# libertininick/imagescry

Hardware: AMD Instinct MI355X
Metric: queries/s cosine top-10 over N x D bank (higher is better)
Workload: dtype f16; 1 GPU; cosine top-10: 1024 fp16 queries x 10000000 x 768 fp16 bank (BASELINE config 4 bank; row-sharded 1 way); bank_rows=10000000, dim=768, queries=1024, k=10, rows_per_gpu=10000000, parallelism=row-shard1

## Files before the change

### imagescry_amd/_lib.py

```python

from __future__ import annotations

import ctypes
import math
import os
from ctypes import POINTER, c_char_p, c_float, c_int, c_int32, c_int64, c_size_t, c_void_p
from pathlib import Path

import torch

LIB_NAME = "libimagescry_hip.so"
LIB_PATH = Path(os.environ.get("ISC_LIB") or Path(__file__).resolve().parent / LIB_NAME)

ISC_U8, ISC_F16, ISC_F32 = 0, 1, 2
ISC_ACT_NONE, ISC_ACT_RELU, ISC_ACT_GELU, ISC_ACT_SILU, ISC_ACT_SIGMOID = 0, 1, 2, 3, 4
ISC_ACT_RESIDUAL_AFTER = 0x100
ISC_TOPK_MAX_K = 120
ISC_SEARCH_MAX_D = 8192
ISC_SEARCH_PASS_QUERIES = 1024
ISC_ABI_VERSION = 4
ISC_BUILD_ABLATION = 1
ISC_GEMM_A_PACKED, ISC_GEMM_W_PACKED, ISC_GEMM_OUT_PACKED, ISC_GEMM_TILE_256, ISC_GEMM_TILE_128 = 1, 2, 4, 8, 16
ISC_KERNEL_DOTS_FILTER, ISC_KERNEL_CONV, ISC_KERNEL_GEMM_F16 = 0, 1, 2

# ... 111 lines not shown
    "isc_im2col_nchw": (
        c_int,
        [c_void_p, c_int, c_int, c_int, c_int, c_int, c_int, c_int, c_int, c_int, c_void_p, c_void_p],
    ),
    "isc_maxpool_nhwc": (c_int, [c_void_p, c_int, c_int, c_int, c_int, c_int, c_int, c_int, c_void_p, c_void_p]),
    "isc_global_avgpool_nhwc": (c_int, [c_void_p, c_int, c_int, c_int, c_int, c_void_p, c_void_p]),
    "isc_pool_linear_l2norm": (
        c_int, [c_void_p, c_int, c_int, c_int, c_int, c_void_p, c_void_p, c_int, c_int, c_float, c_void_p, c_void_p]
    ),
    "isc_gemm_f16": (
        c_int,
        [c_void_p, c_int64, c_int, c_void_p, c_int, c_void_p, c_void_p, c_int, c_void_p, c_int, c_int, c_void_p],
    ),
    "isc_layernorm": (
        c_int,
        [c_void_p, c_int64, c_int, c_int64, c_void_p, c_void_p, c_float, c_void_p, c_int, c_int64, c_int, c_void_p],
    ),
    "isc_attention_f16": (c_int, [c_void_p, c_int, c_int, c_int, c_int, c_void_p, c_int, c_void_p]),
    "isc_patchify_f16": (c_int, [c_void_p, c_int, c_int, c_int, c_int, c_int, c_void_p, c_int, c_void_p]),
    "isc_vit_assemble": (c_int, [c_void_p, c_void_p, c_void_p, c_int, c_int, c_int, c_void_p, c_void_p]),
    "isc_vit_pos_resample": (c_int, [c_void_p, c_int, c_int, c_int, c_int, c_void_p, c_void_p]),
    "isc_vit_tokens_out": (
        c_int, [c_void_p, c_int, c_int, c_int, c_void_p, c_void_p, c_float, c_int, c_float, c_void_p, c_void_p]
    ),
    "isc_cosine_topk_workspace_bytes": (c_int, [c_int, c_int64, c_int, c_int, c_int, POINTER(c_size_t)]),
    "isc_cosine_topk": (
        c_int,
        [c_void_p, c_int, c_int64, c_int, c_void_p, c_int, c_int, c_int64, c_int, c_int64, c_void_p, c_void_p, c_void_p,
         c_void_p, c_void_p, c_size_t, c_void_p],
    ),
    "isc_bank_shadow_bytes": (c_int, [c_int64, c_int, POINTER(c_size_t)]),
    "isc_bank_quantize": (c_int, [c_void_p, c_int64, c_int, c_void_p, c_size_t, c_void_p]),
    "isc_cosine_topk_uses_shadow": (c_int, [c_int, c_int64, c_int, c_int, c_int, POINTER(c_int)]),
    "isc_cosine_topk_shadow": (
        c_int,
        [c_void_p, c_int, c_int64, c_int, c_void_p, c_int, c_int, c_int64, c_int, c_int64, c_void_p, c_void_p, c_void_p,
         c_void_p, c_void_p, c_size_t, c_void_p, c_void_p],
    ),
    "isc_cosine_topk_exhaustive_workspace_bytes": (c_int, [c_int, c_int64, c_int, c_int, c_int, POINTER(c_size_t)]),
    "isc_cosine_topk_exhaustive": (
        c_int,
        [c_void_p, c_int, c_int64, c_int, c_void_p, c_int, c_int, c_int64, c_int, c_int64, c_void_p, c_void_p,
         c_void_p, c_size_t, c_void_p],
    ),
    "isc_cosine_range_workspace_bytes": (c_int, [c_int, c_int64, c_int, c_int, c_int64, POINTER(c_size_t)]),
    "isc_cosine_range": (
        c_int,
        [c_void_p, c_int, c_int64, c_int, c_void_p, c_int, c_int, c_int64, c_void_p, c_int64, c_void_p, c_int64,
         c_void_p, c_void_p, c_void_p, c_void_p, c_void_p, c_void_p, c_size_t, c_void_p],
    ),
    "isc_row_mask_words": (c_int, [c_int64, POINTER(c_size_t)]),
    "isc_row_mask_pack": (c_int, [c_void_p, c_int64, c_void_p, c_void_p, c_void_p]),
    "isc_row_mask_unpack": (c_int, [c_void_p, c_int64, c_int64, c_void_p, c_void_p]),
    "isc_cosine_topk_masked": (
        c_int,
        [c_void_p, c_int, c_int64, c_int, c_void_p, c_int, c_int, c_int64, c_int, c_int64, c_void_p, c_void_p, c_void_p,
         c_void_p, c_void_p, c_size_t, c_void_p, c_void_p],
    ),
    "isc_cosine_topk_exhaustive_masked": (
        c_int,
        [c_void_p, c_int, c_int64, c_int, c_void_p, c_int, c_int, c_int64, c_int, c_int64, c_void_p, c_void_p,
         c_void_p, c_size_t, c_void_p, c_void_p],
    ),
    "isc_cosine_range_masked": (
        c_int,
        [c_void_p, c_int, c_int64, c_int, c_void_p, c_int, c_int, c_int64, c_void_p, c_int64, c_void_p, c_int64,
# ... 130 lines not shown
```

### imagescry_amd/csrc/cosine_topk.hip

```cpp
#include <math.h>
#include <stdlib.h>

#include <type_traits>

#include "bank_layout.h"
#include "isc_common.h"
#include "search_common.h"

namespace {

typedef _Float16 half8 __attribute__((ext_vector_type(8)));
typedef float f32x4 __attribute__((ext_vector_type(4)));
typedef unsigned u32x4 __attribute__((ext_vector_type(4)));
typedef int i32x4 __attribute__((ext_vector_type(4)));

constexpr int TM = 256;
constexpr int NTHREADS = 512;
constexpr int CAP = 32;
constexpr int TARGET_WGS = 256;
constexpr int QCAP = 8192;
constexpr int SLACK = 6;
constexpr int SMALL_Q = 128;
constexpr int QBATCH = ISC_SEARCH_PASS_QUERIES;
constexpr int MAX_LEVELS = 12;
constexpr int SEL_THREADS = 512;
constexpr int SURV_CAP = 2048;
constexpr int TAIL_LCAP = 256;
constexpr int TAIL_COUNT_OFF = 64 * TAIL_LCAP * 8;
constexpr int TAIL_LBOUND_OFF = 140 * 1024;

struct Cand {
    float s;
    int32_t row;
};

struct Level {
    int64_t r0, r1;
    int ntiles, tiles_per_chunk, nchunks;
    int sample;
};

struct Plan {
    int tnq;
    int segs_per_chunk;
    int kp;
    int nslots;
    int qb;
    int qtiles;
    int qpad;
    int max_seg;
    int nlevels;
    int64_t budget;
    Level levels[MAX_LEVELS];
};

int plan_kp(int k) { return (int)isc_align_up((size_t)k + SLACK, 16); }

#ifdef ISC_ABLATION
int forced_tile() {
    static const int v = [] {
        const char* e = getenv("ISC_FORCE_TILE");
        return e ? atoi(e) : 0;
    }();
    return v;
}
#else
constexpr int forced_tile() { return 0; }
#endif

#ifdef ISC_ABLATION
__device__ int g_abl_thr_inf = 0;
int first_ratio() {
    static const int v = getenv("ISC_FIRST_RATIO") ? atoi(getenv("ISC_FIRST_RATIO")) : 16;
    return v;
}
int sample_tiles_cap() {
    static const int v = getenv("ISC_SAMPLE_TILES") ? atoi(getenv("ISC_SAMPLE_TILES")) : 0;
    return v;
}
#else
constexpr int first_ratio() { return 16; }
constexpr int sample_tiles_cap() { return 0; }
#endif

constexpr int COLLAPSE_MIN_KP = 32;
constexpr int COLLAPSE_ROWS_CAP = 64;
constexpr int COLLAPSE_GROUPS = 4096;

Plan make_plan(int64_t n, int q, int k, int group_rows = 0) {
    Plan p;
    p.qb = q < QBATCH ? q : QBATCH;
    p.tnq = p.qb <= 64 ? 64 : p.qb <= SMALL_Q ? 128 : 256;
    if (forced_tile() == 64 || forced_tile() == 128 || forced_tile() == 256) p.tnq = forced_tile();
    p.segs_per_chunk = (8 / (p.tnq / 64)) * 4;
    p.kp = plan_kp(k);
    if (group_rows > 0 && p.kp < COLLAPSE_MIN_KP) p.kp = COLLAPSE_MIN_KP;
    p.qtiles = isc_ceil_div(p.qb, p.tnq);
    p.qpad = p.qtiles * p.tnq;
    p.nslots = group_rows > 0 ? 0 : p.kp <= 16 ? 32 : p.kp <= 32 ? 64 : p.kp <= 64 ? 128 : 0;
    int wgs = TARGET_WGS / p.qtiles;
    if (wgs < 1) wgs = 1;
    const int64_t ntiles_all = isc_ceil_div<int64_t>(n, TM);

    p.nlevels = 0;
    p.max_seg = 0;
    p.budget = 0;
    auto add = [&](int64_t r0, int64_t r1, int sample) {
        Level& l = p.levels[p.nlevels++];
        l.r0 = r0;
        l.r1 = r1;
        l.sample = sample;
        l.ntiles = (int)isc_ceil_div<int64_t>(r1 - r0, TM);
        int want = sample ? l.ntiles : wgs;
        if (want > l.ntiles) want = l.ntiles;
        l.tiles_per_chunk = isc_ceil_div(l.ntiles, want);
        l.nchunks = isc_ceil_div(l.ntiles, l.tiles_per_chunk);
        if (p.segs_per_chunk * l.nchunks > p.max_seg) p.max_seg = p.segs_per_chunk * l.nchunks;
    };
    int64_t stiles = p.nslots ? (int64_t)(QCAP * 7 / 10) / (p.kp * 27 / 20) : 16;
    if (stiles > wgs) stiles = wgs;
    if (sample_tiles_cap() > 0 && stiles > sample_tiles_cap()) stiles = sample_tiles_cap();
    if (stiles < 1) stiles = 1;
    if (stiles > ntiles_all) stiles = ntiles_all;
    int64_t seen = stiles * TM < n ? stiles * TM : n;
    add(0, seen, 1);
    while (seen < n) {
        const int64_t nseg = (int64_t)p.segs_per_chunk * wgs;
        int64_t budget = (int64_t)((double)QCAP * p.kp / (p.kp + 8.0 * sqrt((double)p.kp)));
        if (group_rows > 0) budget = (int64_t)((double)COLLAPSE_GROUPS * p.kp / (p.kp + 8.0 * sqrt((double)p.kp)));
        if (nseg * CAP / 8 < budget) budget = nseg * CAP / 8;
        p.budget = budget;
        const int64_t unit = (int64_t)p.kp * (group_rows > COLLAPSE_ROWS_CAP ? COLLAPSE_ROWS_CAP : group_rows > 0 ? group_rows : 1);
        int64_t ratio = 1 + budget / unit;
        if (p.tnq == 256 && p.qtiles == 1 && p.nlevels == 1 && ratio > first_ratio()) ratio = first_ratio();
        if (ratio < 3) ratio = 3;
        int64_t r1 = seen * ratio;
        if (r1 > n || p.nlevels == MAX_LEVELS - 1) r1 = n;
        add(seen, r1, 0);
        seen = r1;
    }
    const int redo_chunks = (int)(wgs < ntiles_all ? wgs : ntiles_all);
    if (p.segs_per_chunk * redo_chunks > p.max_seg) p.max_seg = p.segs_per_chunk * redo_chunks;
    return p;
}

struct Workspace {
    float* tau;
    float* carry_s;
    int32_t* carry_r;
    int32_t* carry_n;
    int32_t* qflag;
    Cand* seg_ent;
    int32_t* qcount;
    Cand* qlist;
    unsigned char* qpacked;
    int32_t* r_count;
    int32_t* r_list;
    float* tau2;
    int32_t* qcount2;
    int32_t* qflag2;
    unsigned char* qpacked2;
    IscExactWs exact;
    unsigned char* qpacked8;
    float4* qrec8;
    size_t bytes;
};

Workspace carve(const Plan& p, int ks, int64_t n, int k, void* base) {
    Workspace w;
    size_t off = 0;
    auto take = [&](size_t bytes) {
        void* ptr = base ? static_cast<char*>(base) + off : nullptr;
// ... 152 lines not shown
    }
    static __device__ __forceinline__ void row(const u32x4& a0, const u32x4& a1, const u32x4 (&b)[2][4],
                                               f32x4 (&acc)[4]) {
        half(a0, b[0], acc);
        half(a1, b[1], acc);
    }
    template <int N0, int N1>
    static __device__ __forceinline__ void part(const u32x4& a, const u32x4 (&b)[4], f32x4 (&acc)[4]) {
#pragma unroll
        for (int j = 0; j < 4; ++j)
#pragma unroll
            for (int n = N0; n < N1; ++n)
                acc[n] = __builtin_amdgcn_mfma_f32_16x16x4f32(__uint_as_float(a[j]), __uint_as_float(b[n][j]), acc[n],
                                                              0, 0, 0);
    }
};

template <>
struct Mma<signed char> {
    typedef i32x4 Acc;
    template <int N0, int N1>
    static __device__ __forceinline__ void part(const u32x4& a, const u32x4 (&b)[4], i32x4 (&acc)[4]) {
#pragma unroll
        for (int n = N0; n < N1; ++n)
            acc[n] = __builtin_amdgcn_mfma_i32_16x16x64_i8(__builtin_bit_cast(i32x4, a), __builtin_bit_cast(i32x4, b[n]),
                                                           acc[n], 0, 0, 0);
    }
};

struct IscShadowArgs {
    const IscShadowRec* recs;
    const float4* qrec;
};

#define ISC_DS_READ(dst_, addr_, off_) \
    asm volatile("ds_read_b128 %0, %1 offset:%2" : "=v"(dst_) : "v"(addr_), "i"(off_))

__device__ __forceinline__ void glds16(const unsigned char* gsrc, unsigned char* lds_wave_base) {
    __builtin_amdgcn_global_load_lds((const __attribute__((address_space(1))) void*)gsrc,
                                     (__attribute__((address_space(3))) void*)lds_wave_base, 16, 0, 0);
}
template <bool NT>
__device__ __forceinline__ void glds16_bank(const unsigned char* gsrc, unsigned char* lds_wave_base) {
    if constexpr (NT)
        __builtin_amdgcn_global_load_lds((const __attribute__((address_space(1))) void*)gsrc,
                                         (__attribute__((address_space(3))) void*)lds_wave_base, 16, 0, 2);
    else
        glds16(gsrc, lds_wave_base);
}

template <int N>
__device__ __forceinline__ void wait_vmcnt() {
    static_assert(N >= 0 && N <= 63, "vmcnt range");
    asm volatile("s_waitcnt vmcnt(%0)" ::"i"(N) : "memory");
}

constexpr int A_TILE_BYTES = TM * 128;

#ifndef ISC_ASYM_MBLO
#define ISC_ASYM_MBLO 6
#endif
#ifndef ISC_ASYM_SPLIT_MBLO
#define ISC_ASYM_SPLIT_MBLO 8
#endif
#ifndef ISC_HM_RING
#define ISC_HM_RING 4
// ... 566 lines not shown
            asm volatile("s_waitcnt lgkmcnt(0)" : "+v"(ar[cur_][0]), "+v"(ar[cur_][1]));                            \
        __builtin_amdgcn_sched_barrier(0);                                                                           \
        if constexpr (MODE != 3)                                                                                      \
            Mma<T>::row(ar[cur_][0], ar[cur_][1], bq, acc[m_]);                                                      \
        else                                                                                                         \
            acc[m_][0][0] += __uint_as_float(ar[cur_][0][0] ^ ar[cur_][1][1] ^ bq[0][1][0] ^ bq[1][2][1]);           \
    }
            ISC_ROW_STEP(0, 0, 1)
            ISC_ROW_STEP(1, 1, 0)
            ISC_ROW_STEP(2, 0, 1)
            ISC_ROW_STEP(3, 1, 0)
            ISC_ROW_STEP(4, 0, 1)
            ISC_ROW_STEP(5, 1, 0)
            ISC_ROW_STEP(6, 0, 1)
            ISC_ROW_STEP(7, 1, 0)
#undef ISC_ROW_STEP
            }
        }

        }

        if constexpr (!SAMPLE) {
        if (++kt == ksteps) {
            kt = 0;
            constexpr int MBE = STAGGER ? MBHI : MBLO;
            const int64_t trow0 = r0 + (int64_t)(tile_begin + tile) * TM + wave_row0 + fg * 4;
            if constexpr (MASK) {
                if (use_mask) apply_mask(MBE_C{}, SUB_C{}, tile_mask);
            }
            if constexpr (GROUP && !DEFER) apply_codes(MBE_C{}, tile_codes);
            if constexpr (I8) {
                int thr_i[4];
#pragma unroll
                for (int n = 0; n < 4; ++n) {
                    const float t = thr[n] * tile_ct;
                    const float mg = fmaf(qn8[n], tile_et, eq8[n] * (tile_nt + tile_et));
                    const float lo = (t - mg) - (fabsf(t) + mg) * 9.5367431640625e-7f - 1e-30f;
                    thr_i[n] = !(lo <= 2.0e9f) ? INT32_MAX : lo < -2.0e9f ? INT32_MIN : (int)floorf(lo);
                    if (!(tile_nt < INFINITY)) thr_i[n] = thr[n] < INFINITY ? INT32_MIN : INT32_MAX;
                }
                if (r0 + (int64_t)(tile_begin + tile + 1) * TM > r1) {
#pragma unroll
                    for (int m = 0; m < MBE; ++m)
#pragma unroll
                        for (int r = 0; r < 4; ++r)
                            if (trow0 + m * 16 + r >= r1) {
#pragma unroll
                                for (int n = 0; n < 4; ++n) acc[m][n][r] = INT32_MIN;
                            }
                }
#pragma unroll
                for (int n = 0; n < 4; ++n) {
                    int bm[MBE];
                    int mx = INT32_MIN;
#pragma unroll
                    for (int m = 0; m < MBE; ++m) {
                        bm[m] = max(max(acc[m][n][0], acc[m][n][1]), max(acc[m][n][2], acc[m][n][3]));
                        mx = max(mx, bm[m]);
                    }
                    if (__ballot(mx > thr_i[n]) != 0ull) {
#pragma unroll
                        for (int m = 0; m < MBE; ++m) {
                            if (__ballot(bm[m] > thr_i[n]) == 0ull) continue;
#pragma unroll
                            for (int r = 0; r < 4; ++r) {
                                if (acc[m][n][r] > thr_i[n]) {
                                    const int pos = cnt[n]++;
                                    if (pos < CAP)
                                        my_ent[n * 16 * CAP + pos] = Cand{(float)acc[m][n][r], (int32_t)(trow0 + m * 16 + r)};
                                }
                            }
                        }
                    }
// ... 332 lines not shown
}

template <int SPEC>
__global__ __launch_bounds__(SEL_THREADS, 4) void k_select(int32_t* __restrict__ qcount, const Cand* __restrict__ qlist,
                                                        int kp, float* __restrict__ tau, float* __restrict__ carry_s,
                                                        int32_t* __restrict__ carry_r, int32_t* __restrict__ carry_n,
                                                        int32_t* __restrict__ qflag) {
    __shared__ SelShared sh;
    const int q = blockIdx.x;
    const int n = wg_select<SPEC>(sh, q, kp, qcount, qlist, carry_s, carry_r, carry_n);
    const int tid = threadIdx.x;
    if (n < 0) {
        if (tid == 0) {
            qflag[q] = 1;
            tau[q] = INFINITY;
            carry_n[q] = 0;
            qcount[q] = 0;
        }
        return;
    }
    if (tid < n) {
        const unsigned long long key = sh.topk[tid];
        const float sc = isc_key_score(key);
        carry_s[(size_t)q * kp + tid] = sc;
        carry_r[(size_t)q * kp + tid] = isc_key_row(key);
        if (tid == kp - 1) tau[q] = sc;
    }
    if (tid == 0) {
        carry_n[q] = n;
        qcount[q] = 0;
    }
}

__global__ __launch_bounds__(SEL_THREADS, 2) void k_rescore(const unsigned char* __restrict__ bank, int ks,
                                                            const unsigned char* __restrict__ qpacked, int tnq,
                                                            const float* __restrict__ tau, int32_t* __restrict__ qcount,
                                                            Cand* __restrict__ qlist, int64_t nrows) {
    __shared__ float score[QCAP];
    __shared__ int kept;
    const int q = blockIdx.x;
    const int tid = threadIdx.x, lane = tid & 63, wave = tid >> 6;
    constexpr int NW = SEL_THREADS / 64;
    const int n = min(qcount[q], QCAP);
    Cand* list = qlist + (size_t)q * QCAP;
    const unsigned char* qrow_base = qpacked + ((size_t)(q / tnq) * ks * tnq + (q % tnq)) * ISC_KSTEP_BYTES;
    const int nch = ks * 8;
    float qv[2][8];
#pragma unroll
    for (int h = 0; h < 2; ++h) {
        const int ch = lane + 64 * h;
        uint4 raw = make_uint4(0u, 0u, 0u, 0u);
        if (ch < nch) raw = *reinterpret_cast<const uint4*>(qrow_base + (size_t)(ch >> 3) * tnq * ISC_KSTEP_BYTES + (ch & 7) * 16);
        const _Float16* hv = reinterpret_cast<const _Float16*>(&raw);
#pragma unroll
        for (int j = 0; j < 8; ++j) qv[h][j] = (float)hv[j];
    }
    if (tid == 0) kept = 0;
    for (int c0 = wave; c0 < n; c0 += 4 * NW) {
        float acc[4];
#pragma unroll
        for (int u = 0; u < 4; ++u) {
            const int c = c0 + u * NW;
            int row = c < n ? list[c].row : 0;
            if ((unsigned)row >= (unsigned)nrows) row = 0;
            acc[u] = 0.f;
#pragma unroll
            for (int h = 0; h < 2; ++h) {
                const int ch = lane + 64 * h;
                if (ch < nch) {
                    const uint4 raw = *reinterpret_cast<const uint4*>(bank + isc_packed_offset(row, ch >> 3, ks) + (ch & 7) * 16);
                    const _Float16* hv = reinterpret_cast<const _Float16*>(&raw);
#pragma unroll
                    for (int j = 0; j < 8; ++j) acc[u] = fmaf((float)hv[j], qv[h][j], acc[u]);
                }
            }
        }
#pragma unroll
        for (int u = 0; u < 4; ++u) {
            const float tot = isc_wave_sum(acc[u]);
            if (lane == 0 && c0 + u * NW < n) score[c0 + u * NW] = tot;
        }
    }
    __syncthreads();
    const float t = tau[q];
    int rows[SEL_PER];
#pragma unroll
    for (int j = 0; j < SEL_PER; ++j) rows[j] = tid + SEL_THREADS * j < n ? list[tid + SEL_THREADS * j].row : 0;
    __syncthreads();
#pragma unroll
    for (int j = 0; j < SEL_PER; ++j) {
        const int i = tid + SEL_THREADS * j;
        if (i < n && score[i] > t) list[atomicAdd(&kept, 1)] = Cand{score[i], rows[j]};
    }
    __syncthreads();
    if (tid == 0) qcount[q] = kept;
}

template <typename T, typename RowOf, typename Store>
__device__ void exact_dots(const unsigned char* __restrict__ bank, int ks, const unsigned char* qrow_base, int tnq,
                           int nc, int64_t nrows, RowOf row_of, Store store) {
    const int lane = threadIdx.x & 63, wave = threadIdx.x >> 6;
    const int sub = lane >> 3, ch = lane & 7;
    constexpr int NW = SEL_THREADS / 64;
    for (int c0 = wave; c0 < nc; c0 += 4 * NW) {
        int row[4];
        double acc[4];
#pragma unroll
        for (int u = 0; u < 4; ++u) {
            const int c = c0 + u * NW;
            row[u] = c < nc ? row_of(c) : -1;
            if ((unsigned)row[u] >= (unsigned)nrows) row[u] = -1;
            acc[u] = 0.0;
        }
        for (int s0 = 0; s0 < ks; s0 += 8) {
            const int s = s0 + sub;
            if (s < ks) {
                double a[4][8], b[8];
#pragma unroll
                for (int u = 0; u < 4; ++u)
                    Chunk16<T>::load(bank + isc_packed_offset(row[u] < 0 ? 0 : row[u], s, ks) + ch * 16, a[u]);
                Chunk16<T>::load(qrow_base + (size_t)s * tnq * ISC_KSTEP_BYTES + ch * 16, b);
#pragma unroll
                for (int u = 0; u < 4; ++u)
#pragma unroll
                    for (int j = 0; j < Chunk16<T>::N; ++j) acc[u] = fma(a[u][j], b[j], acc[u]);
            }
        }
#pragma unroll
// ... 306 lines not shown
            }
            break;
    }
    }
#undef ISC_LAUNCH_FILTER
}

template <typename F>
void for_each_segment(const Level& l, const Plan& p, F&& launch) {
    int nseg = 1;
    if (!l.sample && p.qtiles > 1) nseg = isc_ceil_div(l.tiles_per_chunk, seg_tiles());
    const int64_t seg_rows = isc_ceil_div<int64_t>(isc_ceil_div<int64_t>(l.r1 - l.r0, nseg), TM) * TM;
    for (int sg = 0; sg < nseg; ++sg) {
        Level ls = l;
        ls.r0 = l.r0 + sg * seg_rows;
        ls.r1 = ls.r0 + seg_rows < l.r1 ? ls.r0 + seg_rows : l.r1;
        if (ls.r0 >= ls.r1) break;
        ls.ntiles = (int)isc_ceil_div<int64_t>(ls.r1 - ls.r0, TM);
        const int want = l.nchunks < ls.ntiles ? l.nchunks : ls.ntiles;
        ls.tiles_per_chunk = isc_ceil_div(ls.ntiles, want);
        ls.nchunks = isc_ceil_div(ls.ntiles, ls.tiles_per_chunk);
        launch(ls);
    }
}

__host__ inline const uint32_t* pass_filter(const uint32_t* m, int, int, const int32_t*) { return m; }
__host__ inline IscGroups pass_filter(IscGroups g, int q0, int q, const int32_t* slots) {
    g.query_group += q0;
    g.nq = q;
    g.slot_query = slots;
    return g;
}

constexpr int I8_INFLATION = 16;
bool plan_uses_i8(const Plan& p, int d) {
    if (p.tnq != 256 || p.qtiles <= 1 || p.nlevels < 3) return false;
    if ((int64_t)isc_shadow_ksteps(d) * ISC_SHADOW_KSTEP_DIMS * 127 * 127 >= (1 << 24)) return false;
    const Level& l = p.levels[p.nlevels - 1];
    return (double)p.kp * (double)(l.r1 - l.r0) / (double)l.r0 * I8_INFLATION <= (double)p.budget;
}

template <typename T, typename TQ, typename... RowMask>
int run(const void* bank, int64_t n, int d, const void* queries, int q_total, int64_t ldq, int k, int64_t index_base,
        const float* norm_bound, float* out_s, int64_t* out_i, int32_t* status, void* ws_base, hipStream_t stream,
        const void* shadow, RowMask... rm) {
    constexpr bool MASK = sizeof...(RowMask) > 0;
    const Plan p = make_plan(n, q_total, k);
    const bool use_i8 = std::is_same<T, _Float16>::value && !MASK && shadow != nullptr && plan_uses_i8(p, d);
#ifdef ISC_ABLATION
    static const bool thr_inf_set = [] {
        const int v = getenv("ISC_THR_INF") != nullptr;
        return hipMemcpyToSymbol(HIP_SYMBOL(g_abl_thr_inf), &v, sizeof(int)) == hipSuccess;
    }();
    (void)thr_inf_set;
#endif
    const int ksteps = isc_ksteps(d, (int)sizeof(T));
    const Workspace w = carve(p, ksteps, n, k, ws_base);
    const unsigned char* bank_bytes = static_cast<const unsigned char*>(bank);
    const IscPerm pm = isc_make_perm(n);
    for (int q0 = 0; q0 < q_total; q0 += p.qb) {
        const int q = q_total - q0 < p.qb ? q_total - q0 : p.qb;
        const TQ* qptr = static_cast<const TQ*>(queries) + (int64_t)q0 * ldq;
        float* os = out_s + (size_t)q0 * k;
        int64_t* oi = out_i + (size_t)q0 * k;
        const bool spec_all = q <= SMALL_Q;
        hipLaunchKernelGGL((k_prep<T, TQ>), dim3(isc_ceil_div(p.qpad * ksteps * 8, 256)), dim3(256), 0, stream, qptr, ldq, q,
                           d, ksteps, p.qpad, p.tnq, w.qpacked, w.tau, w.carry_n, w.qcount, w.qflag,
                           w.exact.redo_count, w.exact.done, w.r_count, w.tau2, w.qcount2, w.qflag2, status,
                           q0 == 0 ? 1 : 0);
        const int ks8 = isc_shadow_ksteps(d);
        if (use_i8)
            hipLaunchKernelGGL((k_prep_i8<TQ>), dim3(p.qpad / 4), dim3(256), 0, stream, qptr, ldq, q, d, ks8, p.tnq,
                               w.qpacked8, w.qrec8);
        const FilterIO io{w.qpacked, w.tau, w.qcount, w.qflag, nullptr};
        for (int li = 0; li < p.nlevels; ++li) {
            const Level& l = p.levels[li];
            if (use_i8 && li == p.nlevels - 1) {
                const unsigned char* sh = static_cast<const unsigned char*>(shadow);
                const IscShadowArgs sa{reinterpret_cast<const IscShadowRec*>(sh + isc_shadow_data_bytes(n, d)), w.qrec8};
                for_each_segment(l, p, [&](const Level& ls) {
                    isc_timing_begin(ISC_KERNEL_DOTS_FILTER, stream);
                    hipLaunchKernelGGL((k_dots_filter<signed char, 256, 12, false, IscShadowArgs>),
                                       dim3(ls.nchunks, p.qtiles), dim3(NTHREADS), 0, stream, sh, ls.r0, ls.r1,
                                       ls.tiles_per_chunk, ls.ntiles, w.qpacked8, ks8, w.tau, p.qpad, w.seg_ent, w.qcount,
                                       w.qlist, p.kp, p.nslots, w.qflag, status, (const int32_t*)nullptr, sa);
                    isc_timing_end(ISC_KERNEL_DOTS_FILTER, stream);
                });
                hipLaunchKernelGGL(k_rescore, dim3(q), dim3(SEL_THREADS), 0, stream, bank_bytes, ksteps, w.qpacked, p.tnq,
                                   w.tau, w.qcount, w.qlist, n);
                continue;
            }
            for_each_segment(l, p, [&](const Level& ls) {
                isc_timing_begin(ISC_KERNEL_DOTS_FILTER, stream);
                if (p.tnq == 256)
                    launch_filter<T, 256>(ls, p, w, io, bank_bytes, ksteps, status, stream,
                                          pass_filter(rm, q0, q, nullptr)...);
                else if (p.tnq == 128)
                    launch_filter<T, 128>(ls, p, w, io, bank_bytes, ksteps, status, stream,
                                          pass_filter(rm, q0, q, nullptr)...);
                else
                    launch_filter<T, 64>(ls, p, w, io, bank_bytes, ksteps, status, stream,
                                         pass_filter(rm, q0, q, nullptr)...);
                isc_timing_end(ISC_KERNEL_DOTS_FILTER, stream);
            });
            if (li + 1 < p.nlevels) {
                if (spec_all)
                    hipLaunchKernelGGL(k_select<SEL_PER>, dim3(q), dim3(SEL_THREADS), 0, stream, w.qcount, w.qlist, p.kp,
                                       w.tau, w.carry_s, w.carry_r, w.carry_n, w.qflag);
                else
                    hipLaunchKernelGGL(k_select<SEL_SPEC_MANY>, dim3(q), dim3(SEL_THREADS), 0, stream, w.qcount, w.qlist,
                                       p.kp, w.tau, w.carry_s, w.carry_r, w.carry_n, w.qflag);
            }
        }
        const RedoLists rl{w.r_count, w.r_list, w.tau2, w.qpacked2, w.exact.redo_count, w.exact.redo_list};
        if (spec_all)
            hipLaunchKernelGGL((k_final<T, SEL_PER, MASK>), dim3(q), dim3(SEL_THREADS), 0, stream, bank_bytes, ksteps, w.qpacked,
                               p.tnq, p.kp, k, pm, index_base, norm_bound, w.qcount, w.qlist, w.carry_s, w.carry_r,
                               w.carry_n, w.qflag, os, oi, rl, status);
        else
            hipLaunchKernelGGL((k_final<T, SEL_SPEC_MANY, MASK>), dim3(q), dim3(SEL_THREADS), 0, stream, bank_bytes, ksteps,
                               w.qpacked, p.tnq, p.kp, k, pm, index_base, norm_bound, w.qcount, w.qlist, w.carry_s,
                               w.carry_r, w.carry_n, w.qflag, os, oi, rl, status);
        {
            const FilterIO rio{w.qpacked2, w.tau2, w.qcount2, w.qflag2, w.r_count};
            Level all;
            all.r0 = 0;
            all.r1 = n;
            all.sample = 0;
            all.ntiles = (int)isc_ceil_div<int64_t>(n, TM);
            int wgs = TARGET_WGS / p.qtiles;
            if (wgs < 1) wgs = 1;
            const int want = wgs < all.ntiles ? wgs : all.ntiles;
            all.tiles_per_chunk = isc_ceil_div(all.ntiles, want);
            all.nchunks = isc_ceil_div(all.ntiles, all.tiles_per_chunk);
            for_each_segment(all, p, [&](const Level& ls) {
                if (p.tnq == 256)
                    launch_filter<T, 256>(ls, p, w, rio, bank_bytes, ksteps, status, stream,
                                          pass_filter(rm, q0, q, w.r_list)...);
                else if (p.tnq == 128)
                    launch_filter<T, 128>(ls, p, w, rio, bank_bytes, ksteps, status, stream,
                                          pass_filter(rm, q0, q, w.r_list)...);
                else
                    launch_filter<T, 64>(ls, p, w, rio, bank_bytes, ksteps, status, stream,
                                         pass_filter(rm, q0, q, w.r_list)...);
            });
            hipLaunchKernelGGL(k_final2<T>, dim3(q), dim3(SEL_THREADS), 0, stream, bank_bytes, ksteps, w.qpacked2, p.tnq, k,
                               pm, index_base, w.r_count, w.r_list, w.qcount2, w.qflag2, w.qlist, os, oi,
                               w.exact.redo_count, w.exact.redo_list, status);
        }
        int st;
        if constexpr (isc_grouped<RowMask...>())
            st = isc_exact_launch(sizeof(T) == 2 ? ISC_F16 : ISC_F32, bank, n, d, qptr, sizeof(TQ) == 2 ? ISC_F16 : ISC_F32,
                                  ldq, k, index_base, w.exact, os, oi, status, pass_filter(rm, q0, q, nullptr)..., stream);
        else
            st = isc_exact_launch(sizeof(T) == 2 ? ISC_F16 : ISC_F32, bank, n, d, qptr,
                                  sizeof(TQ) == 2 ? ISC_F16 : ISC_F32, ldq, k, index_base, w.exact, os, oi, status,
                                  isc_row_mask_ptr(rm...), stream);
        if (st != ISC_OK) return st;
    }
    return isc_launch_status();
}

int check_args(int dtype, int64_t n, int d, int q, int k) {
    if (dtype != ISC_F16 && dtype != ISC_F32) return ISC_ERR_INVALID_ARG;
    if (n <= 0 || d <= 0 || q <= 0 || k <= 0 || k > n) return ISC_ERR_INVALID_ARG;
    if (k > ISC_TOPK_MAX_K) return ISC_ERR_UNSUPPORTED;
    if (n > 0x7ffffffe) return ISC_ERR_UNSUPPORTED;
    if (d > ISC_SEARCH_MAX_D) return ISC_ERR_UNSUPPORTED;
    if (q > ISC_SEARCH_MAX_Q) return ISC_ERR_UNSUPPORTED;
    return ISC_OK;
}

}

extern "C" int isc_cosine_topk_workspace_bytes(int dtype, int64_t N, int D, int Q, int k, size_t* bytes) {
    ISC_REQUIRE(bytes);
    const int st = check_args(dtype, N, D, Q, k);
    if (st != ISC_OK) return st;
    *bytes = carve(make_plan(N, Q, k), isc_ksteps(D, dtype == ISC_F16 ? 2 : 4), N, k, nullptr).bytes;
    return ISC_OK;
}

namespace {

int topk(const void* bank, int dtype, int64_t N, int D, const void* queries, int q_dtype, int Q, int64_t ldq, int k,
         int64_t index_base, const float* norm_bound, float* out_scores, int64_t* out_indices, int32_t* status,
         void* workspace, size_t workspace_bytes, const uint32_t* row_mask, void* stream,
         const IscGroups* groups = nullptr, const void* shadow = nullptr) {
    ISC_REQUIRE(bank && queries && out_scores && out_indices && status);
    ISC_REQUIRE(q_dtype == ISC_F16 || q_dtype == ISC_F32);
    const int st = check_args(dtype, N, D, Q, k);
    if (st != ISC_OK) return st;
// ... 12 lines not shown
    if (dtype == ISC_F16) {
        if (q_dtype == ISC_F16) ISC_RUN(_Float16, _Float16);
        ISC_RUN(_Float16, float);
    }
    if (q_dtype == ISC_F16) ISC_RUN(float, _Float16);
    ISC_RUN(float, float);
#undef ISC_RUN
}

}

extern "C" int isc_cosine_topk(const void* bank, int dtype, int64_t N, int D, const void* queries, int q_dtype, int Q,
                               int64_t ldq, int k, int64_t index_base, const float* norm_bound, float* out_scores,
                               int64_t* out_indices, int32_t* status, void* workspace, size_t workspace_bytes,
                               void* stream) {
    return topk(bank, dtype, N, D, queries, q_dtype, Q, ldq, k, index_base, norm_bound, out_scores, out_indices, status,
                workspace, workspace_bytes, nullptr, stream);
}

extern "C" int isc_cosine_topk_shadow(const void* bank, int dtype, int64_t N, int D, const void* queries, int q_dtype,
                                      int Q, int64_t ldq, int k, int64_t index_base, const float* norm_bound,
                                      float* out_scores, int64_t* out_indices, int32_t* status, void* workspace,
                                      size_t workspace_bytes, const void* shadow, void* stream) {
    ISC_REQUIRE(dtype == ISC_F16 || shadow == nullptr);
    if (!isc_aligned(shadow, 256)) return ISC_ERR_ALIGNMENT;
    return topk(bank, dtype, N, D, queries, q_dtype, Q, ldq, k, index_base, norm_bound, out_scores, out_indices, status,
                workspace, workspace_bytes, nullptr, stream, nullptr, shadow);
}

extern "C" int isc_cosine_topk_uses_shadow(int dtype, int64_t N, int D, int Q, int k, int* uses) {
    ISC_REQUIRE(uses);
    const int st = check_args(dtype, N, D, Q, k);
    if (st != ISC_OK) return st;
    *uses = dtype == ISC_F16 && plan_uses_i8(make_plan(N, Q, k), D) ? 1 : 0;
    return ISC_OK;
}

extern "C" int isc_cosine_topk_masked(const void* bank, int dtype, int64_t N, int D, const void* queries, int q_dtype,
                                      int Q, int64_t ldq, int k, int64_t index_base, const float* norm_bound,
                                      float* out_scores, int64_t* out_indices, int32_t* status, void* workspace,
                                      size_t workspace_bytes, const uint32_t* row_mask, void* stream) {
    ISC_REQUIRE(row_mask);
    return topk(bank, dtype, N, D, queries, q_dtype, Q, ldq, k, index_base, norm_bound, out_scores, out_indices, status,
                workspace, workspace_bytes, row_mask, stream);
}

extern "C" int isc_cosine_topk_grouped(const void* bank, int dtype, int64_t N, int D, const void* queries, int q_dtype,
                                       int Q, int64_t ldq, int k, int64_t index_base, const float* norm_bound,
                                       float* out_scores, int64_t* out_indices, int32_t* status, void* workspace,
                                       size_t workspace_bytes, const uint32_t* row_mask, const int32_t* row_group,
                                       const int32_t* query_group, void* stream) {
    ISC_REQUIRE(row_group && query_group);
    if (!isc_aligned(row_group, 16) || !isc_aligned(query_group, 4) || !isc_aligned(row_mask, 4))
        return ISC_ERR_ALIGNMENT;
    const IscGroups g{row_mask, row_group, query_group, nullptr, Q};
    return topk(bank, dtype, N, D, queries, q_dtype, Q, ldq, k, index_base, norm_bound, out_scores, out_indices, status,
                workspace, workspace_bytes, row_mask, stream, &g);
}

namespace {

constexpr int GH = COLLAPSE_GROUPS;
constexpr int GH_PER = GH / SEL_THREADS;
constexpr int GH_EMPTY = INT32_MIN;
static_assert(GH % SEL_THREADS == 0 && GH_PER <= SEL_PER && GH == 4096, "hash slots per thread; 12-bit hash");

struct GroupHash {
// ... 526 lines not shown
```

### include/imagescry_hip.h

```cpp
#ifndef IMAGESCRY_HIP_H
#define IMAGESCRY_HIP_H

#include <stddef.h>
#include <stdint.h>

#ifdef __cplusplus
extern "C" {
#endif

#define ISC_ABI_VERSION 4

#define ISC_U8 0
#define ISC_F16 1
#define ISC_F32 2

#define ISC_OK 0
#define ISC_ERR_INVALID_ARG (-1)
#define ISC_ERR_UNSUPPORTED (-2)
#define ISC_ERR_WORKSPACE (-3)
#define ISC_ERR_LAUNCH (-4)
#define ISC_ERR_NO_DEVICE (-5)
#define ISC_ERR_ALIGNMENT (-6)

#define ISC_ACT_NONE 0
// ... 125 lines not shown
int isc_patchify_f16(const float* x, int B, int C, int H, int W, int patch, void* patches, int packed, void* stream);

int isc_vit_assemble(const float* patch_embed, const float* cls_token, const float* pos_embed, int B, int T, int D,
                     float* tokens, void* stream);

int isc_vit_pos_resample(const float* pos_embed, int g, int h, int w, int D, float* out, void* stream);

int isc_vit_tokens_out(const float* tokens, int B, int T, int D, const float* gamma, const float* beta, float eps,
                       int normalize, float l2_eps, float* out, void* stream);


int isc_feature_sums_workspace_bytes(int64_t n, int F, size_t* bytes);
int isc_feature_sums(const float* x, int64_t n, int F, int64_t ldx, double* sums, void* workspace, size_t workspace_bytes,
                     void* stream);

int isc_center_transpose(const float* x, int64_t n, int F, int64_t ldx, const float* mean, float* xt, int Fpad,
                         int64_t ldn, void* stream);

int isc_gram_rows(const float* xt, int F, int64_t n, float* gram, void* stream);


#define ISC_TOPK_MAX_K 120
#define ISC_SEARCH_MAX_D 8192
#define ISC_SEARCH_MAX_Q (1 << 24)
#define ISC_SEARCH_PASS_QUERIES 1024
int isc_cosine_topk_workspace_bytes(int dtype, int64_t N, int D, int Q, int k, size_t* bytes);
int isc_cosine_topk(const void* bank, int dtype, int64_t N, int D, const void* queries, int q_dtype, int Q, int64_t ldq,
                    int k, int64_t index_base, const float* norm_bound, float* out_scores, int64_t* out_indices,
                    int32_t* status, void* workspace, size_t workspace_bytes, void* stream);

int isc_bank_shadow_bytes(int64_t N, int D, size_t* bytes);
int isc_bank_quantize(const void* packed, int64_t N, int D, void* shadow, size_t shadow_bytes, void* stream);
int isc_cosine_topk_uses_shadow(int dtype, int64_t N, int D, int Q, int k, int* uses);
int isc_cosine_topk_shadow(const void* bank, int dtype, int64_t N, int D, const void* queries, int q_dtype, int Q,
                           int64_t ldq, int k, int64_t index_base, const float* norm_bound, float* out_scores,
                           int64_t* out_indices, int32_t* status, void* workspace, size_t workspace_bytes,
                           const void* shadow, void* stream);

int isc_cosine_topk_masked(const void* bank, int dtype, int64_t N, int D, const void* queries, int q_dtype, int Q,
                           int64_t ldq, int k, int64_t index_base, const float* norm_bound, float* out_scores,
                           int64_t* out_indices, int32_t* status, void* workspace, size_t workspace_bytes,
                           const uint32_t* row_mask, void* stream);

int isc_cosine_topk_grouped(const void* bank, int dtype, int64_t N, int D, const void* queries, int q_dtype, int Q,
                            int64_t ldq, int k, int64_t index_base, const float* norm_bound, float* out_scores,
                            int64_t* out_indices, int32_t* status, void* workspace, size_t workspace_bytes,
                            const uint32_t* row_mask, const int32_t* row_group, const int32_t* query_group, void* stream);

int isc_cosine_topk_exhaustive_workspace_bytes(int dtype, int64_t N, int D, int Q, int k, size_t* bytes);
int isc_cosine_topk_exhaustive(const void* bank, int dtype, int64_t N, int D, const void* queries, int q_dtype, int Q,
                               int64_t ldq, int k, int64_t index_base, float* out_scores, int64_t* out_indices,
                               void* workspace, size_t workspace_bytes, void* stream);

int isc_cosine_topk_exhaustive_masked(const void* bank, int dtype, int64_t N, int D, const void* queries, int q_dtype,
                                      int Q, int64_t ldq, int k, int64_t index_base, float* out_scores,
                                      int64_t* out_indices, void* workspace, size_t workspace_bytes,
                                      const uint32_t* row_mask, void* stream);

int isc_cosine_topk_exhaustive_grouped(const void* bank, int dtype, int64_t N, int D, const void* queries, int q_dtype,
                                       int Q, int64_t ldq, int k, int64_t index_base, float* out_scores,
                                       int64_t* out_indices, void* workspace, size_t workspace_bytes,
                                       const uint32_t* row_mask, const int32_t* row_group, const int32_t* query_group,
                                       void* stream);

int isc_cosine_scores(const void* bank, int dtype, int64_t capacity, int D, const void* queries, int q_dtype, int Q,
                      int64_t ldq, const int64_t* rows, int64_t M, const uint32_t* fill_mask, float* scores, int64_t lds,
// ... 47 lines not shown
```

Before: 123,000 queries/s.

## Run int8 shadow filtering on all levels after the first, with two-stage rescore

The level planner now lays out geometric row ranges sized so that every level after the first can use the int8 shadow bank filter, with the first non-sample level kept in fp16 by default. Before, only the last level could use int8. The rescore kernel becomes two-stage: it first re-scores a small top set of approximate candidates exactly to tighten the threshold, then fetches fp16 rows only for candidates whose int8 score can still beat that threshold. This cuts fp16 bank traffic and rescore work, at the cost of more planning complexity, extra rescore launches per level and more selection work inside k_rescore. A plan-query API and ablation counters are also added.

```diff
diff --git a/imagescry_amd/_lib.py b/imagescry_amd/_lib.py
--- a/imagescry_amd/_lib.py
+++ b/imagescry_amd/_lib.py
@@ -167,6 +167,10 @@
     "isc_bank_shadow_bytes": (c_int, [c_int64, c_int, POINTER(c_size_t)]),
     "isc_bank_quantize": (c_int, [c_void_p, c_int64, c_int, c_void_p, c_size_t, c_void_p]),
     "isc_cosine_topk_uses_shadow": (c_int, [c_int, c_int64, c_int, c_int, c_int, POINTER(c_int)]),
+    "isc_cosine_topk_plan": (
+        c_int,
+        [c_int, c_int64, c_int, c_int, c_int, c_int, c_int, POINTER(c_int), POINTER(c_int64), POINTER(c_int)],
+    ),
     "isc_cosine_topk_shadow": (
         c_int,
         [c_void_p, c_int, c_int64, c_int, c_void_p, c_int, c_int, c_int64, c_int, c_int64, c_void_p, c_void_p, c_void_p,
diff --git a/imagescry_amd/csrc/cosine_topk.hip b/imagescry_amd/csrc/cosine_topk.hip
--- a/imagescry_amd/csrc/cosine_topk.hip
+++ b/imagescry_amd/csrc/cosine_topk.hip
@@ -1,4 +1,5 @@
 #include <math.h>
+#include <stdio.h>
 #include <stdlib.h>
 
 #include <type_traits>
@@ -38,6 +39,7 @@
     int64_t r0, r1;
     int ntiles, tiles_per_chunk, nchunks;
     int sample;
+    int kind;
 };
 
 struct Plan {
@@ -82,12 +84,30 @@
 constexpr int first_ratio() { return 16; }
 constexpr int sample_tiles_cap() { return 0; }
 #endif
+#ifdef ISC_ABLATION
+bool i8_first_piece_i8() {
+    static const bool v = getenv("ISC_I8_FIRST_I8") != nullptr;
+    return v;
+}
+#else
+constexpr bool i8_first_piece_i8() { return false; }
+#endif
+#ifdef ISC_ABLATION
+bool i8_last_level_only() {
+    static const bool v = getenv("ISC_I8_LAST_ONLY") != nullptr;
+    return v;
+}
+#else
+constexpr bool i8_last_level_only() { return false; }
+#endif
 
 constexpr int COLLAPSE_MIN_KP = 32;
 constexpr int COLLAPSE_ROWS_CAP = 64;
 constexpr int COLLAPSE_GROUPS = 4096;
 
-Plan make_plan(int64_t n, int q, int k, int group_rows = 0) {
+constexpr int I8_INFLATION = 16;
+
+Plan make_plan(int64_t n, int q, int k, int group_rows = 0, bool i8 = false) {
     Plan p;
     p.qb = q < QBATCH ? q : QBATCH;
     p.tnq = p.qb <= 64 ? 64 : p.qb <= SMALL_Q ? 128 : 256;
@@ -110,6 +130,7 @@
         l.r0 = r0;
         l.r1 = r1;
         l.sample = sample;
+        l.kind = sample ? 0 : 1;
         l.ntiles = (int)isc_ceil_div<int64_t>(r1 - r0, TM);
         int want = sample ? l.ntiles : wgs;
         if (want > l.ntiles) want = l.ntiles;
@@ -124,6 +145,7 @@
     if (stiles > ntiles_all) stiles = ntiles_all;
     int64_t seen = stiles * TM < n ? stiles * TM : n;
     add(0, seen, 1);
+    const int64_t seen0 = seen;
     while (seen < n) {
         const int64_t nseg = (int64_t)p.segs_per_chunk * wgs;
         int64_t budget = (int64_t)((double)QCAP * p.kp / (p.kp + 8.0 * sqrt((double)p.kp)));
@@ -138,6 +160,57 @@
         if (r1 > n || p.nlevels == MAX_LEVELS - 1) r1 = n;
         add(seen, r1, 0);
         seen = r1;
+    }
+    if (i8 && group_rows == 0 && p.tnq == 256 && p.qtiles > 1 && p.nlevels > 1) {
+        const Plan flt = p;
+        const int64_t list_budget = (int64_t)((double)QCAP * p.kp / (p.kp + 8.0 * sqrt((double)p.kp)));
+        auto level_budget = [&](int nchunks) {
+            const int64_t slots = (int64_t)p.segs_per_chunk * nchunks * CAP / 8;
+            return slots < list_budget ? slots : list_budget;
+        };
+        auto chunks_of = [&](int64_t r0, int64_t r1) {
+            const int ntiles = (int)isc_ceil_div<int64_t>(r1 - r0, TM);
+            const int per = isc_ceil_div(ntiles, wgs < ntiles ? wgs : ntiles);
+            return isc_ceil_div(ntiles, per);
+        };
+        auto fits_i8 = [&](int64_t r0, int64_t r1) {
+            return (double)p.kp * (double)(r1 - r0) / (double)r0 * I8_INFLATION <= (double)level_budget(chunks_of(r0, r1));
+        };
+        const int64_t r8 = 1 + level_budget(wgs) / ((int64_t)p.kp * I8_INFLATION);
+        int64_t ends[MAX_LEVELS];
+        int m = 0;
+        bool ok = r8 >= 2 && !i8_last_level_only();
+        for (int64_t b = n; ok && b > seen0;) {
+            if (m == MAX_LEVELS - 1) {
+                ok = false;
+                break;
+            }
+            ends[m++] = b;
+            int64_t nb = isc_ceil_div<int64_t>(isc_ceil_div<int64_t>(b, r8), TM) * TM;
+            for (int it = 0; it < 64 && nb < b && nb > seen0 && !fits_i8(nb, b); ++it) {
+                const int64_t r = 1 + level_budget(chunks_of(nb, b)) / ((int64_t)p.kp * I8_INFLATION);
+                const int64_t up = isc_ceil_div<int64_t>(isc_ceil_div<int64_t>(b, r), TM) * TM;
+                nb = up > nb ? up : nb + TM;
+            }
+            if (nb >= b) ok = false;
+            b = nb;
+        }
+        if (ok) {
+            p.nlevels = 1;
+            for (int j = m - 1; j >= 0; --j) {
+                add(p.levels[p.nlevels - 1].r1, ends[j], 0);
+                Level& l = p.levels[p.nlevels - 1];
+                if (fits_i8(l.r0, l.r1)) l.kind = 2;
+                else ok = false;
+            }
+            if (ok && !i8_first_piece_i8() && p.nlevels > 2) p.levels[1].kind = 1;
+        }
+        if (!ok) {
+            p = flt;
+            Level& l = p.levels[p.nlevels - 1];
+            if (p.nlevels >= 3 && (double)p.kp * (double)(l.r1 - l.r0) / (double)l.r0 * I8_INFLATION <= (double)p.budget)
+                l.kind = 2;
+        }
     }
     const int redo_chunks = (int)(wgs < ntiles_all ? wgs : ntiles_all);
     if (p.segs_per_chunk * redo_chunks > p.max_seg) p.max_seg = p.segs_per_chunk * redo_chunks;
@@ -356,6 +429,15 @@
     const IscShadowRec* recs;
     const float4* qrec;
 };
+
+__device__ __forceinline__ int isc_i8_threshold(float thr_cq, float ct, float et, float nt, float qn, float eq) {
+    const float t = thr_cq * ct;
+    const float mg = fmaf(qn, et, eq * (nt + et));
+    const float lo = (t - mg) - (fabsf(t) + mg) * 9.5367431640625e-7f - 1e-30f;
+    int r = !(lo <= 2.0e9f) ? INT32_MAX : lo < -2.0e9f ? INT32_MIN : (int)floorf(lo);
+    if (!(nt < INFINITY)) r = thr_cq < INFINITY ? INT32_MIN : INT32_MAX;
+    return r;
+}
 
 #define ISC_DS_READ(dst_, addr_, off_) \
     asm volatile("ds_read_b128 %0, %1 offset:%2" : "=v"(dst_) : "v"(addr_), "i"(off_))
@@ -988,13 +1070,7 @@
             if constexpr (I8) {
                 int thr_i[4];
 #pragma unroll
-                for (int n = 0; n < 4; ++n) {
-                    const float t = thr[n] * tile_ct;
-                    const float mg = fmaf(qn8[n], tile_et, eq8[n] * (tile_nt + tile_et));
-                    const float lo = (t - mg) - (fabsf(t) + mg) * 9.5367431640625e-7f - 1e-30f;
-                    thr_i[n] = !(lo <= 2.0e9f) ? INT32_MAX : lo < -2.0e9f ? INT32_MIN : (int)floorf(lo);
-                    if (!(tile_nt < INFINITY)) thr_i[n] = thr[n] < INFINITY ? INT32_MIN : INT32_MAX;
-                }
+                for (int n = 0; n < 4; ++n) thr_i[n] = isc_i8_threshold(thr[n], tile_ct, tile_et, tile_nt, qn8[n], eq8[n]);
                 if (r0 + (int64_t)(tile_begin + tile + 1) * TM > r1) {
 #pragma unroll
                     for (int m = 0; m < MBE; ++m)
@@ -1393,68 +1469,157 @@
     }
 }
 
-__global__ __launch_bounds__(SEL_THREADS, 2) void k_rescore(const unsigned char* __restrict__ bank, int ks,
-                                                            const unsigned char* __restrict__ qpacked, int tnq,
-                                                            const float* __restrict__ tau, int32_t* __restrict__ qcount,
-                                                            Cand* __restrict__ qlist, int64_t nrows) {
-    __shared__ float score[QCAP];
-    __shared__ int kept;
-    const int q = blockIdx.x;
-    const int tid = threadIdx.x, lane = tid & 63, wave = tid >> 6;
+#ifdef ISC_ABLATION
+__device__ unsigned long long g_abl_rescore[4];
+#endif
+constexpr int RS_PMAX = ISC_TOPK_MAX_K + 8;
+
+template <int RS_ROWS, typename Store>
+__device__ __forceinline__ void rescore_rows(const unsigned char* __restrict__ bank, int ks, const float (&qv)[2][8],
+                                             const int* prow, int np, int64_t nrows, Store store) {
+    const int lane = threadIdx.x & 63, wave = threadIdx.x >> 6;
     constexpr int NW = SEL_THREADS / 64;
-    const int n = min(qcount[q], QCAP);
-    Cand* list = qlist + (size_t)q * QCAP;
-    const unsigned char* qrow_base = qpacked + ((size_t)(q / tnq) * ks * tnq + (q % tnq)) * ISC_KSTEP_BYTES;
     const int nch = ks * 8;
-    float qv[2][8];
-#pragma unroll
-    for (int h = 0; h < 2; ++h) {
-        const int ch = lane + 64 * h;
-        uint4 raw = make_uint4(0u, 0u, 0u, 0u);
-        if (ch < nch) raw = *reinterpret_cast<const uint4*>(qrow_base + (size_t)(ch >> 3) * tnq * ISC_KSTEP_BYTES + (ch & 7) * 16);
-        const _Float16* hv = reinterpret_cast<const _Float16*>(&raw);
-#pragma unroll
-        for (int j = 0; j < 8; ++j) qv[h][j] = (float)hv[j];
-    }
-    if (tid == 0) kept = 0;
-    for (int c0 = wave; c0 < n; c0 += 4 * NW) {
-        float acc[4];
-#pragma unroll
-        for (int u = 0; u < 4; ++u) {
+    for (int c0 = wave; c0 < np; c0 += RS_ROWS * NW) {
+        int row[RS_ROWS];
+        uint4 raw[RS_ROWS][2];
+#pragma unroll
+        for (int u = 0; u < RS_ROWS; ++u) {
             const int c = c0 + u * NW;
-            int row = c < n ? list[c].row : 0;
-            if ((unsigned)row >= (unsigned)nrows) row = 0;
-            acc[u] = 0.f;
+            row[u] = c < np ? prow[c] : 0;
+            if ((unsigned)row[u] >= (unsigned)nrows) row[u] = 0;
+        }
+#pragma unroll
+        for (int u = 0; u < RS_ROWS; ++u)
 #pragma unroll
             for (int h = 0; h < 2; ++h) {
                 const int ch = lane + 64 * h;
-                if (ch < nch) {
-                    const uint4 raw = *reinterpret_cast<const uint4*>(bank + isc_packed_offset(row, ch >> 3, ks) + (ch & 7) * 16);
-                    const _Float16* hv = reinterpret_cast<const _Float16*>(&raw);
-#pragma unroll
-                    for (int j = 0; j < 8; ++j) acc[u] = fmaf((float)hv[j], qv[h][j], acc[u]);
-                }
-            }
-        }
-#pragma unroll
-        for (int u = 0; u < 4; ++u) {
-            const float tot = isc_wave_sum(acc[u]);
-            if (lane == 0 && c0 + u * NW < n) score[c0 + u * NW] = tot;
-        }
-    }
-    __syncthreads();
+                raw[u][h] = make_uint4(0u, 0u, 0u, 0u);
+                if (ch < nch && c0 + u * NW < np)
+                    raw[u][h] = *reinterpret_cast<const uint4*>(bank + isc_packed_offset(row[u], ch >> 3, ks) + (ch & 7) * 16);
+            }
+#pragma unroll
+        for (int u = 0; u < RS_ROWS; ++u) {
+            float acc = 0.f;
+#pragma unroll
+            for (int h = 0; h < 2; ++h) {
+                const _Float16* hv = reinterpret_cast<const _Float16*>(&raw[u][h]);
+#pragma unroll
+                for (int j = 0; j < 8; ++j) acc = fmaf((float)hv[j], qv[h][j], acc);
+            }
+            const float tot = isc_wave_sum(acc);
+            if (lane == 0 && c0 + u * NW < np) store(c0 + u * NW, row[u], tot);
+        }
+    }
+}
+
+__global__ __launch_bounds__(SEL_THREADS, 2) void k_rescore(const unsigned char* __restrict__ bank, int ks,
+                                                            const unsigned char* __restrict__ qpacked, int tnq, int kp,
+                                                            const float* __restrict__ tau,
+                                                            const float* __restrict__ carry_s,
+                                                            const int32_t* __restrict__ carry_n, IscShadowArgs sa,
+                                                            int32_t* __restrict__ qcount, Cand* __restrict__ qlist,
+                                                            int64_t nrows) {
+    __shared__ SelShared sh;
+    __shared__ int prow[QCAP];
+    __shared__ float vals[RS_PMAX + ISC_TOPK_MAX_K + 8];
+    __shared__ float tau2_sh;
+    __shared__ int kept, npend;
+    const int q = blockIdx.x;
+    const int tid = threadIdx.x, lane = tid & 63;
+    const int n = min(qcount[q], QCAP);
+    if (n == 0) return;
+    Cand* list = qlist + (size_t)q * QCAP;
     const float t = tau[q];
-    int rows[SEL_PER];
-#pragma unroll
-    for (int j = 0; j < SEL_PER; ++j) rows[j] = tid + SEL_THREADS * j < n ? list[tid + SEL_THREADS * j].row : 0;
-    __syncthreads();
+    const float4 qr = sa.qrec[q];
+    const int nc = min(carry_n[q], kp);
+    const int ptarget = min(2 * kp, RS_PMAX);
+
+    int eacc[SEL_PER];
+    unsigned long long key[SEL_PER + 1];
 #pragma unroll
     for (int j = 0; j < SEL_PER; ++j) {
         const int i = tid + SEL_THREADS * j;
-        if (i < n && score[i] > t) list[atomicAdd(&kept, 1)] = Cand{score[i], rows[j]};
-    }
+        Cand e{0.f, 0};
+        if (i < n) e = list[i];
+        if ((unsigned)e.row >= (unsigned)nrows) e.row = 0;
+        eacc[j] = (int)e.s;
+        IscShadowRec r{1.f, 1.f, 0.f, 0.f};
+        if (i < n) r = sa.recs[e.row >> 8];
+        const float approx = e.s / (qr.x * r.inv_scale);
+        key[j] = i < n ? isc_make_key(approx == approx && r.qnorm < INFINITY ? approx : -INFINITY, e.row) : 0ull;
+    }
+    key[SEL_PER] = 0ull;
+    float qv[2][8];
+    {
+        const unsigned char* qrow_base = qpacked + ((size_t)(q / tnq) * ks * tnq + (q % tnq)) * ISC_KSTEP_BYTES;
+#pragma unroll
+        for (int h = 0; h < 2; ++h) {
+            const int ch = lane + 64 * h;
+            uint4 raw = make_uint4(0u, 0u, 0u, 0u);
+            if (ch < ks * 8) raw = *reinterpret_cast<const uint4*>(qrow_base + (size_t)(ch >> 3) * tnq * ISC_KSTEP_BYTES + (ch & 7) * 16);
+            const _Float16* hv = reinterpret_cast<const _Float16*>(&raw);
+#pragma unroll
+            for (int j = 0; j < 8; ++j) qv[h][j] = (float)hv[j];
+        }
+    }
+    if (tid == 0) {
+        kept = 0;
+        npend = 0;
+    }
+
+    const int nsel = wg_select_keys(sh, key, ptarget);
+    const int np = nsel < 0 ? 0 : nsel;
+    const unsigned long long pkey = np > 0 ? sh.topk[np - 1] : ~0ull;
+    if (tid < np) prow[tid] = isc_key_row(sh.topk[tid]);
+    if (tid < nc) vals[RS_PMAX + tid] = carry_s[(size_t)q * kp + tid];
+    __syncthreads();
+    rescore_rows<4>(bank, ks, qv, prow, np, nrows, [&](int i, int row, float s) {
+        vals[i] = s;
+        if (s > t) list[atomicAdd(&kept, 1)] = Cand{s, row};
+    });
+    __syncthreads();
+    const int nv = np + nc;
+    if (tid == 0) tau2_sh = t;
+    __syncthreads();
+    if (nv >= kp && tid < nv) {
+        auto val = [&](int i) {
+            const float v = vals[i < np ? i : RS_PMAX + (i - np)];
+            return v == v ? v : -INFINITY;
+        };
+        const float mine = val(tid);
+        int rank = 0;
+        for (int j = 0; j < nv; ++j) {
+            const float o = val(j);
+            rank += (o > mine || (o == mine && j < tid)) ? 1 : 0;
+        }
+        if (rank == kp - 1) tau2_sh = fmaxf(t, mine);
+    }
+    __syncthreads();
+    const float t2 = tau2_sh;
+
+    const float t2c = t2 * qr.x;
+#pragma unroll
+    for (int j = 0; j < SEL_PER; ++j) {
+        if (key[j] == 0ull || key[j] >= pkey) continue;
+        const int row = isc_key_row(key[j]);
+        const IscShadowRec r = sa.recs[row >> 8];
+        if (eacc[j] > isc_i8_threshold(t2c, r.inv_scale, r.resid, r.qnorm, qr.y, qr.z)) prow[atomicAdd(&npend, 1)] = row;
+    }
+    __syncthreads();
+    rescore_rows<8>(bank, ks, qv, prow, npend, nrows, [&](int, int row, float s) {
+        if (s > t) list[atomicAdd(&kept, 1)] = Cand{s, row};
+    });
     __syncthreads();
     if (tid == 0) qcount[q] = kept;
+#ifdef ISC_ABLATION
+    if (tid == 0) {
+        atomicAdd(&g_abl_rescore[0], (unsigned long long)n);
+        atomicAdd(&g_abl_rescore[1], (unsigned long long)np);
+        atomicAdd(&g_abl_rescore[2], (unsigned long long)npend);
+        atomicAdd(&g_abl_rescore[3], 1ull);
+    }
+#endif
 }
 
 template <typename T, typename RowOf, typename Store>
@@ -1827,12 +1992,11 @@
     return g;
 }
 
-constexpr int I8_INFLATION = 16;
-bool plan_uses_i8(const Plan& p, int d) {
-    if (p.tnq != 256 || p.qtiles <= 1 || p.nlevels < 3) return false;
-    if ((int64_t)isc_shadow_ksteps(d) * ISC_SHADOW_KSTEP_DIMS * 127 * 127 >= (1 << 24)) return false;
-    const Level& l = p.levels[p.nlevels - 1];
-    return (double)p.kp * (double)(l.r1 - l.r0) / (double)l.r0 * I8_INFLATION <= (double)p.budget;
+bool i8_dims_ok(int d) { return (int64_t)isc_shadow_ksteps(d) * ISC_SHADOW_KSTEP_DIMS * 127 * 127 < (1 << 24); }
+bool plan_has_i8(const Plan& p) {
+    for (int li = 0; li < p.nlevels; ++li)
+        if (p.levels[li].kind == 2) return true;
+    return false;
 }
 
 template <typename T, typename TQ, typename... RowMask>
@@ -1840,8 +2004,8 @@
         const float* norm_bound, float* out_s, int64_t* out_i, int32_t* status, void* ws_base, hipStream_t stream,
         const void* shadow, RowMask... rm) {
     constexpr bool MASK = sizeof...(RowMask) > 0;
-    const Plan p = make_plan(n, q_total, k);
-    const bool use_i8 = std::is_same<T, _Float16>::value && !MASK && shadow != nullptr && plan_uses_i8(p, d);
+    const Plan p = make_plan(n, q_total, k, 0, std::is_same<T, _Float16>::value && !MASK && shadow != nullptr && i8_dims_ok(d));
+    const bool use_i8 = plan_has_i8(p);
 #ifdef ISC_ABLATION
     static const bool thr_inf_set = [] {
         const int v = getenv("ISC_THR_INF") != nullptr;
@@ -1870,7 +2034,7 @@
         const FilterIO io{w.qpacked, w.tau, w.qcount, w.qflag, nullptr};
         for (int li = 0; li < p.nlevels; ++li) {
             const Level& l = p.levels[li];
-            if (use_i8 && li == p.nlevels - 1) {
+            if (l.kind == 2) {
                 const unsigned char* sh = static_cast<const unsigned char*>(shadow);
                 const IscShadowArgs sa{reinterpret_cast<const IscShadowRec*>(sh + isc_shadow_data_bytes(n, d)), w.qrec8};
                 for_each_segment(l, p, [&](const Level& ls) {
@@ -1882,22 +2046,22 @@
                     isc_timing_end(ISC_KERNEL_DOTS_FILTER, stream);
                 });
                 hipLaunchKernelGGL(k_rescore, dim3(q), dim3(SEL_THREADS), 0, stream, bank_bytes, ksteps, w.qpacked, p.tnq,
-                                   w.tau, w.qcount, w.qlist, n);
-                continue;
-            }
-            for_each_segment(l, p, [&](const Level& ls) {
-                isc_timing_begin(ISC_KERNEL_DOTS_FILTER, stream);
-                if (p.tnq == 256)
-                    launch_filter<T, 256>(ls, p, w, io, bank_bytes, ksteps, status, stream,
-                                          pass_filter(rm, q0, q, nullptr)...);
-                else if (p.tnq == 128)
-                    launch_filter<T, 128>(ls, p, w, io, bank_bytes, ksteps, status, stream,
-                                          pass_filter(rm, q0, q, nullptr)...);
-                else
-                    launch_filter<T, 64>(ls, p, w, io, bank_bytes, ksteps, status, stream,
-                                         pass_filter(rm, q0, q, nullptr)...);
-                isc_timing_end(ISC_KERNEL_DOTS_FILTER, stream);
-            });
+                                   p.kp, w.tau, w.carry_s, w.carry_n, sa, w.qcount, w.qlist, n);
+            } else {
+                for_each_segment(l, p, [&](const Level& ls) {
+                    isc_timing_begin(ISC_KERNEL_DOTS_FILTER, stream);
+                    if (p.tnq == 256)
+                        launch_filter<T, 256>(ls, p, w, io, bank_bytes, ksteps, status, stream,
+                                              pass_filter(rm, q0, q, nullptr)...);
+                    else if (p.tnq == 128)
+                        launch_filter<T, 128>(ls, p, w, io, bank_bytes, ksteps, status, stream,
+                                              pass_filter(rm, q0, q, nullptr)...);
+                    else
+                        launch_filter<T, 64>(ls, p, w, io, bank_bytes, ksteps, status, stream,
+                                             pass_filter(rm, q0, q, nullptr)...);
+                    isc_timing_end(ISC_KERNEL_DOTS_FILTER, stream);
+                });
+            }
             if (li + 1 < p.nlevels) {
                 if (spec_all)
                     hipLaunchKernelGGL(k_select<SEL_PER>, dim3(q), dim3(SEL_THREADS), 0, stream, w.qcount, w.qlist, p.kp,
@@ -1953,6 +2117,17 @@
                                   isc_row_mask_ptr(rm...), stream);
         if (st != ISC_OK) return st;
     }
+#ifdef ISC_ABLATION
+    if (use_i8 && getenv("ISC_RESCORE_COUNT")) {
+        unsigned long long c[4] = {0, 0, 0, 0};
+        const unsigned long long zero[4] = {0, 0, 0, 0};
+        if (hipStreamSynchronize(stream) == hipSuccess &&
+            hipMemcpyFromSymbol(c, HIP_SYMBOL(g_abl_rescore), sizeof(c)) == hipSuccess && c[3] > 0)
+            fprintf(stderr, "k_rescore per query and level: %.1f entries, %.1f rows fetched in stage A, %.1f in stage B (%llu)\n",
+                    (double)c[0] / c[3], (double)c[1] / c[3], (double)c[2] / c[3], c[3]);
+        (void)hipMemcpyToSymbol(HIP_SYMBOL(g_abl_rescore), zero, sizeof(zero));
+    }
+#endif
     return isc_launch_status();
 }
 
@@ -2031,7 +2206,22 @@
     ISC_REQUIRE(uses);
     const int st = check_args(dtype, N, D, Q, k);
     if (st != ISC_OK) return st;
-    *uses = dtype == ISC_F16 && plan_uses_i8(make_plan(N, Q, k), D) ? 1 : 0;
+    *uses = plan_has_i8(make_plan(N, Q, k, 0, dtype == ISC_F16 && i8_dims_ok(D))) ? 1 : 0;
+    return ISC_OK;
+}
+
+extern "C" int isc_cosine_topk_plan(int dtype, int64_t N, int D, int Q, int k, int shadow, int max_levels, int* nlevels,
+                                    int64_t* row_end, int* kind) {
+    ISC_REQUIRE(nlevels && row_end && kind && max_levels >= 0);
+    const int st = check_args(dtype, N, D, Q, k);
+    if (st != ISC_OK) return st;
+    const Plan p = make_plan(N, Q, k, 0, shadow != 0 && dtype == ISC_F16 && i8_dims_ok(D));
+    *nlevels = p.nlevels;
+    if (p.nlevels > max_levels) return ISC_ERR_INVALID_ARG;
+    for (int li = 0; li < p.nlevels; ++li) {
+        row_end[li] = p.levels[li].r1;
+        kind[li] = p.levels[li].kind;
+    }
     return ISC_OK;
 }
 
diff --git a/include/imagescry_hip.h b/include/imagescry_hip.h
--- a/include/imagescry_hip.h
+++ b/include/imagescry_hip.h
@@ -181,6 +181,8 @@
 int isc_bank_shadow_bytes(int64_t N, int D, size_t* bytes);
 int isc_bank_quantize(const void* packed, int64_t N, int D, void* shadow, size_t shadow_bytes, void* stream);
 int isc_cosine_topk_uses_shadow(int dtype, int64_t N, int D, int Q, int k, int* uses);
+int isc_cosine_topk_plan(int dtype, int64_t N, int D, int Q, int k, int shadow, int max_levels, int* nlevels,
+                         int64_t* row_end, int* kind);
 int isc_cosine_topk_shadow(const void* bank, int dtype, int64_t N, int D, const void* queries, int q_dtype, int Q,
                            int64_t ldq, int k, int64_t index_base, const float* norm_bound, float* out_scores,
                            int64_t* out_indices, int32_t* status, void* workspace, size_t workspace_bytes,
```

Measured after the change: 138,600 queries/s, median of 6. 12.7% higher.
